# davidesantangelo/krep

Measured on NVIDIA H100. Metric: GB/s scanned (HBM-resident corpus), higher is better.
Workload: dtype u8

## Files before the change

krep_b200/csrc/scan_count.cu:

```cuda
#include <algorithm>
#include "engine.h"
#include "line_rec.cuh"
#include "lit_filters.cuh"

namespace kb {

struct CountDev
{
    LitDevParams p;
    uint64_t own_end;
    uint32_t part_groups, n_parts;
    uint32_t exact;
    uint32_t tail;
    LineRec *recs;
};

struct PartState
{
    uint32_t lines = 0;
    bool has_hit = false, first_open = false, pending = false, seen_nl = false;
    uint64_t covered_to = 0;
};

__device__ __noinline__ unsigned verify_exact_call(const LitDevParams &p, long long cand) { return verify_exact(p, cand); }

__device__ __noinline__ bool scan_for_newline(const LitDevParams &p, uint64_t lo, uint64_t hi)
{
    const uint32_t lane = threadIdx.x & 31;
    if (hi > p.avail_len) hi = p.avail_len;
    for (uint64_t base = lo & ~15ull; base < hi; base += 512)
    {
        const uint64_t unit = base + 16ull * lane;
        uint32_t nm = 0;
        if (unit < hi && unit + 16 > lo)
        {
            if (unit + 16 <= p.avail_len) nm = nl_mask16(__ldg(reinterpret_cast<const uint4 *>(p.text + unit)));
            else
                for (uint64_t q = unit; q < p.avail_len; q++) nm |= (p.text[q] == '\n' ? 1u : 0u) << (uint32_t)(q - unit);
            nm &= range_mask16(unit, lo, hi);
        }
        if (__any_sync(0xffffffffu, nm != 0)) return true;
    }
    return false;
}

__device__ __forceinline__ void settle(const LitDevParams &p, PartState &S, uint64_t upto)
{
    if (S.covered_to < upto && (S.pending || (!S.has_hit && !S.seen_nl)))
        if (scan_for_newline(p, S.covered_to, upto))
        {
            S.pending = false;
            S.seen_nl = true;
        }
}

__device__ __forceinline__ void account(PartState &S, uint32_t hm, uint32_t nm)
{
    const uint32_t lane = threadIdx.x & 31;
    const bool has_nl = nm != 0;
    const uint32_t fnl = has_nl ? (uint32_t)__ffs(nm) - 1 : 0, lnl = has_nl ? 31u - (uint32_t)__clz(nm) : 0;
    const bool f = has_nl && (hm & ((1u << fnl) - 1u)) != 0;
    const bool l = has_nl && ((hm >> lnl) >> 1) != 0;
    uint32_t inner = 0;
    if (__popc(nm) >= 2)
    {
        uint32_t prev = fnl, rest = nm & (nm - 1);
        while (rest)
        {
            const uint32_t nx = (uint32_t)__ffs(rest) - 1;
            if (hm & (((1u << nx) - 1u) & ~((2u << prev) - 1u))) inner++;
            prev = nx;
            rest &= rest - 1;
        }
    }
    const uint32_t A = __ballot_sync(0xffffffffu, has_nl), T = __ballot_sync(0xffffffffu, !has_nl && hm != 0);
    const uint32_t F = __ballot_sync(0xffffffffu, f), Lm = __ballot_sync(0xffffffffu, l);
    uint32_t innersum = 0;
    if (__ballot_sync(0xffffffffu, inner != 0)) innersum = __reduce_add_sync(0xffffffffu, inner);
    if (A == 0)
    {
        if (T)
        {
            if (!S.pending)
            {
                S.lines++;
                if (!S.has_hit && !S.seen_nl) S.first_open = true;
            }
            S.pending = true;
            S.has_hit = true;
        }
        return;
    }
    const uint32_t j1 = (uint32_t)__ffs(A) - 1, jr = 31u - (uint32_t)__clz(A);
    if ((T & ((1u << j1) - 1u)) || ((F >> j1) & 1u))
    {
        if (!S.pending)
        {
            S.lines++;
            if (!S.has_hit && !S.seen_nl) S.first_open = true;
        }
        S.has_hit = true;
    }
    S.pending = false;
    S.seen_nl = true;
    bool gap = false;
    if (has_nl && lane != j1)
    {
        const uint32_t below = A & ((1u << lane) - 1u);
        const uint32_t pj = 31u - (uint32_t)__clz(below);
        const uint32_t between = ((1u << lane) - 1u) & ~((2u << pj) - 1u);
        gap = ((Lm >> pj) & 1u) || (T & between) || f;
    }
    const uint32_t G = __ballot_sync(0xffffffffu, gap);
    S.lines += (uint32_t)__popc(G) + innersum;
    if (G || innersum) S.has_hit = true;
    if (((Lm >> jr) & 1u) || ((T >> jr) >> 1))
    {
        S.lines++;
        S.has_hit = true;
        S.pending = true;
    }
}

__device__ __forceinline__ uint64_t pack_state(const PartState &S)
{
    return (uint64_t)S.lines | ((uint64_t)((S.has_hit ? 1u : 0u) | (S.first_open ? 2u : 0u) | (S.pending ? 4u : 0u) | (S.seen_nl ? 8u : 0u)) << 32);
}
__device__ __forceinline__ void unpack_state(uint64_t k, PartState &S)
{
    S.lines = (uint32_t)k;
    const uint32_t f = (uint32_t)(k >> 32);
    S.has_hit = f & 1u;
    S.first_open = f & 2u;
    S.pending = f & 4u;
    S.seen_nl = f & 8u;
}
__device__ __noinline__ uint64_t account_call(uint64_t packed, uint32_t hm, uint32_t nm)
{
    PartState S;
    unpack_state(packed, S);
    account(S, hm, nm);
    return pack_state(S);
}

template <bool WINDOW>
__device__ __noinline__ uint32_t hit_mask16(const CountDev &D, uint64_t unit, const uint4 &v, uint32_t nx)
{
    const LitDevParams &p = D.p;
    const uint32_t w[5] = {v.x, v.y, v.z, v.w, nx};
    uint32_t hm = 0;
    if (WINDOW)
    {
        const uint32_t mask = p.fold & p.win_mask, k0 = p.K[0];
#pragma unroll
        for (int k = 0; k < 4; k++)
#pragma unroll
            for (int r = 0; r < 4; r++)
            {
                const uint32_t win = r == 0 ? w[k] : __funnelshift_r(w[k], w[k + 1], 8 * r);
                if ((win & mask) == k0)
                {
                    const uint64_t st = unit + 4 * k + r;
                    const bool ok = D.exact ? (st >= p.own_begin && st < p.own_end && st + p.m <= p.avail_len)
                                            : verify_exact_call(p, (long long)st) != 0;
                    if (ok) hm |= 1u << (4 * k + r);
                }
            }
    }
    else
    {
#pragma unroll
        for (int k = 0; k < 4; k++)
#pragma unroll
            for (int d = 0; d < 4; d++)
                if ((w[k] & p.fold) == p.K[d] && verify_exact_call(p, (long long)(unit + 4 * k) - d)) hm |= 1u << (4 * k);
    }
    return hm;
}

__device__ __noinline__ PartState count_tail(const CountDev &D, PartState S, uint64_t cov, uint64_t nl_lo, uint64_t nl_hi, bool window)
{
    const LitDevParams &p = D.p;
    const uint32_t lane = threadIdx.x & 31;
    if (p.avail_len < p.emit_len && cov >= nl_hi) return S;
    const uint64_t last_start = p.avail_len >= p.emit_len ? p.avail_len - p.emit_len : 0;
    uint64_t end = nl_hi > last_start + 1 ? nl_hi : last_start + 1;
    if (!window && end < cov + 1) end = cov + 1;
    for (uint64_t base = cov; base < end; base += 32)
    {
        settle(p, S, base > nl_lo ? base : nl_lo);
        const uint64_t q = base + lane;
        uint32_t hm = 0, nm = 0;
        if (q < end)
        {
            if (p.avail_len >= p.emit_len && q >= p.tail_start && q <= last_start && verify_exact(p, (long long)q)) hm = 1;
            if (!window && q == cov && p.avail_len >= p.emit_len)
                for (uint64_t s = p.tail_start; s < cov && s <= last_start; s++)
                    if (verify_exact(p, (long long)s)) hm = 1;
            if (q >= nl_lo && q < nl_hi && q < p.avail_len && p.text[q] == '\n') nm = 1;
            if (nm) hm = 0;
        }
        account(S, hm, nm);
        S.covered_to = base + 32;
    }
    return S;
}

#ifndef KREP_B200_COUNT_MINB
#define KREP_B200_COUNT_MINB 3
#endif
template <bool WINDOW, bool FOLD, bool MASKED>
__global__ void __launch_bounds__(256, KREP_B200_COUNT_MINB) k_count_lines(const __grid_constant__ CountDev D)
{
    const LitDevParams &p = D.p;
    const uint4 *__restrict__ t4 = reinterpret_cast<const uint4 *>(p.text);
    const uint32_t lane = threadIdx.x & 31;
    const uint32_t warp_global = (blockIdx.x * blockDim.x + threadIdx.x) >> 5, total_warps = (gridDim.x * blockDim.x) >> 5;
    const uint32_t k0 = p.K[0], k1 = p.K[1], k2 = p.K[2], k3 = p.K[3], fold = p.fold, mask = p.win_mask;
    const uint32_t c1 = p.mulc[0], c2 = p.mulc[1], c3 = p.mulc[2];
    for (uint32_t pi = warp_global; pi < D.n_parts; pi += total_warps)
    {
        const uint64_t ga = p.group_begin + (uint64_t)pi * D.part_groups;
        uint64_t gb = ga + D.part_groups;
        if (gb > p.group_end) gb = p.group_end;
        const bool last_part = pi + 1 == D.n_parts;
        const uint64_t nl_lo = ga * 16 > p.own_begin ? ga * 16 : p.own_begin;
        const uint64_t nl_hi = (last_part || gb * 16 > D.own_end) ? D.own_end : gb * 16;
        PartState S;
        S.covered_to = nl_lo;
        for (uint64_t g = ga; g < gb; g += 128)
        {
            uint4 v[4];
            uint32_t nx[4];
            bool ok[4];
#pragma unroll
            for (int u = 0; u < 4; u++)
            {
                const uint64_t gi = g + 32 * u + lane;
                ok[u] = gi < gb;
                v[u] = ok[u] ? ld_stream(t4 + gi) : make_uint4(0u, 0u, 0u, 0u);
                nx[u] = 0;
                if (WINDOW && ok[u] && (lane == 31 || gi + 1 >= gb)) nx[u] = __ldg(reinterpret_cast<const uint32_t *>(t4 + gi + 1));
            }
            uint32_t cand = 0;
#pragma unroll
            for (int u = 0; u < 4; u++)
            {
                bool h;
                if (WINDOW)
                {
                    const uint32_t nb = __shfl_down_sync(0xffffffffu, v[u].x, 1);
                    if (!(lane == 31 || g + 32 * u + lane + 1 >= gb)) nx[u] = nb;
                    h = hit_vec_w<FOLD, MASKED>(v[u], nx[u], fold, mask, k0, c1, c2, c3);
                }
                else
                    h = hit_vec<FOLD>(v[u], fold, k0, k1, k2, k3);
                cand |= (h && ok[u]) ? (1u << u) : 0u;
            }
            const uint32_t any = __reduce_or_sync(0xffffffffu, cand);
            if (any)
            {
                const uint64_t tile_lo = g * 16;
                settle(p, S, tile_lo > nl_lo ? tile_lo : nl_lo);
                const bool inside = tile_lo >= nl_lo && tile_lo + 2048 <= nl_hi;
                uint64_t st = pack_state(S);
#pragma unroll
                for (int u = 0; u < 4; u++)
                {
                    const uint64_t unit = tile_lo + 512ull * u + 16ull * lane;
                    uint32_t hm = 0, nm = 0;
                    if (ok[u])
                    {
                        if ((cand >> u) & 1u) hm = hit_mask16<WINDOW>(D, unit, v[u], nx[u]);
                        nm = nl_mask16(v[u]);
                        if (!inside) nm &= range_mask16(unit, nl_lo, nl_hi);
                    }
                    st = account_call(st, hm, nm);
                }
                unpack_state(st, S);
                S.covered_to = tile_lo + 2048;
            }
        }
        if (last_part && D.tail) S = count_tail(D, S, gb * 16, nl_lo, nl_hi, WINDOW);
        uint32_t flags = 0;
        if (S.has_hit)
        {
            if (S.pending && S.covered_to < nl_hi && scan_for_newline(p, S.covered_to, nl_hi)) S.pending = false;
            flags = LR_HAS_HIT | (S.first_open ? LR_FIRST_OPEN : 0u) | (S.pending ? LR_LAST_PENDING : 0u) | LR_HAS_NL;
        }
        else
        {
            const bool nl = S.seen_nl || (S.covered_to < nl_hi && scan_for_newline(p, S.covered_to, nl_hi));
            flags = nl ? LR_HAS_NL : 0u;
        }
        if (lane == 0) D.recs[pi] = LineRec{S.lines, flags};
    }
}

__global__ void __launch_bounds__(1024) k_count_finish(const LineRec *recs, uint32_t n, uint64_t *d_out, uint64_t *h_out)
{
    __shared__ uint64_t s_lines[1024];
    __shared__ uint32_t s_flags[1024];
    const uint32_t per = (n + blockDim.x - 1) / blockDim.x;
    const uint32_t a = threadIdx.x * per, b = a + per < n ? a + per : n;
    uint64_t lines = 0;
    uint32_t flags = 0;
    for (uint32_t i = a; i < b; i++) append_rec(lines, flags, recs[i].lines, recs[i].flags);
    s_lines[threadIdx.x] = lines;
    s_flags[threadIdx.x] = flags;
    __syncthreads();
    if (threadIdx.x == 0)
    {
        lines = 0;
        flags = 0;
        for (uint32_t t = 0; t < blockDim.x; t++) append_rec(lines, flags, s_lines[t], s_flags[t]);
        d_out[0] = lines;
        d_out[1] = flags;
        h_out[0] = lines;
        h_out[1] = flags;
    }
}

#define CKC(call)                                                                                  \
    do                                                                                             \
    {                                                                                              \
        cudaError_t e_ = (call);                                                                   \
        if (e_ != cudaSuccess)                                                                     \
        {                                                                                          \
            set_error(-2, "CUDA error %s at %s:%d (%s)", cudaGetErrorName(e_), __FILE__, __LINE__, \
                      cudaGetErrorString(e_));                                                     \
            return -2;                                                                             \
        }                                                                                          \
    } while (0)

bool count_lines_eligible(const Plan *plan, const search_params_t *P, int algo)
{
    if (!P->count_lines_mode || plan->is_regex || plan->whole_word == 2) return false;
    if (plan->is_ac)
    {
        for (const std::string &s : plan->patterns)
            if (s.find('\n') != std::string::npos) return false;
        return true;
    }
    if (plan->emit_len != plan->m) return false;
    if (plan->pattern.find('\n') != std::string::npos) return false;
    return algo == KREP_B200_ALGO_BMH || algo == KREP_B200_ALGO_KMP || algo == KREP_B200_ALGO_MEMCHR ||
           algo == KREP_B200_ALGO_MEMCHR_SHORT || algo == KREP_B200_ALGO_SSE42;
}

int ensure_line_out(DevCtx &E, uint64_t n)
{
    if (n <= E.line_out_cap) return 0;
    CKC(cudaDeviceSynchronize());
    cudaFree(E.d_line_out);
    cudaFreeHost(E.h_line_out);
    E.d_line_out = nullptr;
    E.h_line_out = nullptr;
    E.line_out_cap = 0;
    uint64_t cap = 64;
    while (cap < n) cap *= 2;
    CKC(cudaMalloc(&E.d_line_out, cap * 2 * sizeof(uint64_t)));
    CKC(cudaHostAlloc(&E.h_line_out, cap * 2 * sizeof(uint64_t), cudaHostAllocMapped | cudaHostAllocPortable));
    E.line_out_cap = cap;
    return 0;
}

int launch_count_lines(DevCtx &E, const Plan *plan, const krep_b200_shard_t *sh, cudaStream_t stream, uint64_t index)
{
    if (((uintptr_t)sh->d_text & 15) != 0)
    {
        set_error(-3, "shard text pointer must be 16-byte aligned");
        return -3;
    }
    const PlanDev *pd = plan_on_device(plan, E);
    if (!pd) return -2;
    if (ensure_line_out(E, index + 1) != 0) return -2;
    if (plan->is_ac)
    {
        const int slot = set_count_slot(E);
        const int rc = set_count_begin(E, plan, sh, stream, slot);
        return rc != 0 ? rc : set_count_end(E, plan, sh, stream, slot, index);
    }
    CountDev D;
    memset(&D, 0, sizeof D);
    LitDevParams &p = D.p;
    const uint64_t own_end = sh->own_end < sh->avail_len ? sh->own_end : sh->avail_len;
    p.text = (const uint8_t *)sh->d_text;
    p.avail_len = sh->avail_len;
    p.own_begin = sh->own_begin;
    p.own_end = own_end;
    p.global_offset = sh->global_offset;
    p.prev_byte = sh->prev_byte;
    p.next_byte = sh->next_byte;
    uint64_t total_groups;
    const bool window = plan->filter == FILTER_WINDOW4;
    if (!window)
    {
        total_groups = sh->avail_len / 16;
        p.tail_start = total_groups ? total_groups * 16 - 3 : 0;
    }
    else
    {
        total_groups = sh->avail_len >= 20 ? (sh->avail_len - 20) / 16 + 1 : 0;
        p.tail_start = total_groups * 16;
    }
    p.group_begin = sh->own_begin / 16;
    p.group_end = (own_end + 2) / 16 + 1;
    D.tail = p.group_end > total_groups ? 1u : 0u;
    if (p.group_end > total_groups) p.group_end = total_groups;
    if (p.group_begin > p.group_end) p.group_begin = p.group_end;
    p.m = plan->m;
    p.emit_len = plan->emit_len;
    for (int d = 0; d < 4; d++) p.K[d] = plan->K[d];
    p.fold = plan->fold;
    p.win_mask = plan->win_mask;
    p.mulc[0] = 1u << 24;
    p.mulc[1] = 1u << 16;
    p.mulc[2] = 1u << 8;
    p.pat_val = pd->d_pat_val;
    p.pat_mask = pd->d_pat_mask;
    p.whole_word = plan->whole_word;
    D.own_end = own_end;
    {
        bool letters = true;
        for (unsigned char ch : plan->pattern) letters &= is_alpha_c(ch);
        D.exact = (window && plan->m <= 4 && plan->whole_word == 0 && (plan->case_sensitive || letters)) ? 1u : 0u;
    }
    const uint64_t groups = p.group_end - p.group_begin;
    const char *v = getenv("KREP_B200_COUNT_PART_KB");
    const uint32_t kb_ = v && atoi(v) > 0 ? (uint32_t)atoi(v) : 64;
    uint64_t part = std::max<uint32_t>(128, kb_ * 64 / 128 * 128);
    const uint64_t max_parts = 1u << 18;
    if ((groups + part - 1) / part > max_parts) part = ((groups + max_parts - 1) / max_parts + 127) / 128 * 128;
    D.part_groups = (uint32_t)part;
    D.n_parts = (uint32_t)std::max<uint64_t>((groups + part - 1) / part, 1);
    if (D.n_parts > E.line_recs_cap)
    {
        CKC(cudaStreamSynchronize(stream));
        cudaFree(E.d_line_recs);
        E.d_line_recs = nullptr;
        E.line_recs_cap = 0;
        const uint64_t cap = std::max<uint64_t>(D.n_parts, 1u << 16);
        CKC(cudaMalloc(&E.d_line_recs, cap * sizeof(LineRec)));
        E.line_recs_cap = cap;
    }
    D.recs = (LineRec *)E.d_line_recs;
    const bool folded = plan->fold != 0xFFFFFFFFu, masked = plan->win_mask != 0xFFFFFFFFu;
    const uint64_t want_blocks = ((uint64_t)D.n_parts + 7) / 8;
    const unsigned grid = (unsigned)std::min<uint64_t>(want_blocks, (uint64_t)E.sm_count * KREP_B200_COUNT_MINB);
    if (!window)
    {
        if (folded) k_count_lines<false, true, false><<<grid, 256, 0, stream>>>(D);
        else k_count_lines<false, false, false><<<grid, 256, 0, stream>>>(D);
    }
    else if (folded)
    {
        if (masked) k_count_lines<true, true, true><<<grid, 256, 0, stream>>>(D);
        else k_count_lines<true, true, false><<<grid, 256, 0, stream>>>(D);
    }
    else
    {
        if (masked) k_count_lines<true, false, true><<<grid, 256, 0, stream>>>(D);
        else k_count_lines<true, false, false><<<grid, 256, 0, stream>>>(D);
    }
    CKC(cudaGetLastError());
    k_count_finish<<<1, 1024, 0, stream>>>(D.recs, D.n_parts, E.d_line_out + 2 * index, E.h_line_out + 2 * index);
    CKC(cudaGetLastError());
    count_launch(2);
    return 0;
}

uint64_t combine_line_records(const uint64_t *recs, size_t n)
{
    uint64_t lines = 0;
    uint32_t flags = 0;
    for (size_t i = 0; i < n; i++) append_rec(lines, flags, recs[2 * i], (uint32_t)recs[2 * i + 1]);
    return lines;
}

}
```

Before: 3123.

## Rewrite line counting with a bitwise carry-propagation formula and prefetch loads

Replaces the branchy per-warp line-accounting state machine, including its newline rescans and packed-state noinline calls, with a compact carry-based formula. Per-lane hit masks are combined with newline masks through an addition trick, and the carry between lanes and iterations comes from ballots. The loop also double-buffers the next tile's vector loads, computes window hits as full masks, and verifies candidates bit by bit. Tiles with no hits only run a cheap newline test. This cuts instruction count and serialization in the count kernel, but relies on subtle bit arithmetic that must match the old semantics at part boundaries.

```diff
diff --git a/krep_b200/csrc/scan_count.cu b/krep_b200/csrc/scan_count.cu
--- a/krep_b200/csrc/scan_count.cu
+++ b/krep_b200/csrc/scan_count.cu
@@ -9,176 +9,103 @@
 {
     LitDevParams p;
     uint64_t own_end;
+    uint64_t hit_hi;
     uint32_t part_groups, n_parts;
     uint32_t exact;
     uint32_t tail;
     LineRec *recs;
 };
 
-struct PartState
-{
-    uint32_t lines = 0;
-    bool has_hit = false, first_open = false, pending = false, seen_nl = false;
-    uint64_t covered_to = 0;
+struct CountState
+{
+    uint32_t lines;
+    uint32_t carry;
+    uint32_t seen;
+    uint32_t first_open;
 };
 
 __device__ __noinline__ unsigned verify_exact_call(const LitDevParams &p, long long cand) { return verify_exact(p, cand); }
 
-__device__ __noinline__ bool scan_for_newline(const LitDevParams &p, uint64_t lo, uint64_t hi)
-{
-    const uint32_t lane = threadIdx.x & 31;
-    if (hi > p.avail_len) hi = p.avail_len;
-    for (uint64_t base = lo & ~15ull; base < hi; base += 512)
-    {
-        const uint64_t unit = base + 16ull * lane;
-        uint32_t nm = 0;
-        if (unit < hi && unit + 16 > lo)
+__device__ __forceinline__ void account(CountState &S, uint32_t hm, uint32_t nm, uint32_t lanes_below)
+{
+    const uint32_t ev = hm | nm;
+    const uint32_t E = __ballot_sync(0xffffffffu, ev != 0);
+    const uint32_t N = __ballot_sync(0xffffffffu, nm > hm);
+    const uint32_t eb = E & lanes_below, nb = N & lanes_below;
+    const uint32_t cin = eb ? (nb > (eb ^ nb) ? 1u : 0u) : S.carry;
+    S.lines += __popc((((nm << 1) | cin) + (~ev & 0xFFFFu)) & hm);
+    if (E != 0 && !S.seen)
+    {
+        const uint32_t F = __ballot_sync(0xffffffffu, (ev & (0u - ev) & hm) != 0);
+        S.first_open = (F & E & (0u - E)) ? 1u : 0u;
+        S.seen = 1;
+    }
+    S.carry = E ? (N > (E ^ N) ? 1u : 0u) : S.carry;
+}
+
+__device__ __forceinline__ bool has_nl16(const uint4 &v)
+{
+    const uint32_t x0 = v.x ^ 0x0A0A0A0Au, x1 = v.y ^ 0x0A0A0A0Au, x2 = v.z ^ 0x0A0A0A0Au, x3 = v.w ^ 0x0A0A0A0Au;
+    const uint32_t z = ((x0 - 0x01010101u) & ~x0) | ((x1 - 0x01010101u) & ~x1) | ((x2 - 0x01010101u) & ~x2) |
+                       ((x3 - 0x01010101u) & ~x3);
+    return (z & 0x80808080u) != 0;
+}
+
+template <bool FOLD, bool MASKED>
+__device__ __forceinline__ uint32_t window_hits16(const uint4 &v, uint32_t nx, uint32_t fold, uint32_t mask, uint32_t k0,
+                                                  uint32_t c1, uint32_t c2, uint32_t c3)
+{
+    uint32_t w[5] = {v.x, v.y, v.z, v.w, nx};
+    uint32_t hm = 0;
+#pragma unroll
+    for (int k = 0; k < 4; k++)
+    {
+        uint32_t lo = w[k], hi = w[k + 1];
+        if (FOLD)
         {
-            if (unit + 16 <= p.avail_len) nm = nl_mask16(__ldg(reinterpret_cast<const uint4 *>(p.text + unit)));
-            else
-                for (uint64_t q = unit; q < p.avail_len; q++) nm |= (p.text[q] == '\n' ? 1u : 0u) << (uint32_t)(q - unit);
-            nm &= range_mask16(unit, lo, hi);
+            lo &= fold;
+            hi &= fold;
         }
-        if (__any_sync(0xffffffffu, nm != 0)) return true;
-    }
-    return false;
-}
-
-__device__ __forceinline__ void settle(const LitDevParams &p, PartState &S, uint64_t upto)
-{
-    if (S.covered_to < upto && (S.pending || (!S.has_hit && !S.seen_nl)))
-        if (scan_for_newline(p, S.covered_to, upto))
+        uint32_t x0 = lo, x1 = hi * c1 + __umulhi(lo, c1), x2 = hi * c2 + __umulhi(lo, c2), x3 = hi * c3 + __umulhi(lo, c3);
+        if (MASKED)
         {
-            S.pending = false;
-            S.seen_nl = true;
+            x0 &= mask; x1 &= mask; x2 &= mask; x3 &= mask;
         }
-}
-
-__device__ __forceinline__ void account(PartState &S, uint32_t hm, uint32_t nm)
-{
-    const uint32_t lane = threadIdx.x & 31;
-    const bool has_nl = nm != 0;
-    const uint32_t fnl = has_nl ? (uint32_t)__ffs(nm) - 1 : 0, lnl = has_nl ? 31u - (uint32_t)__clz(nm) : 0;
-    const bool f = has_nl && (hm & ((1u << fnl) - 1u)) != 0;
-    const bool l = has_nl && ((hm >> lnl) >> 1) != 0;
-    uint32_t inner = 0;
-    if (__popc(nm) >= 2)
-    {
-        uint32_t prev = fnl, rest = nm & (nm - 1);
-        while (rest)
-        {
-            const uint32_t nx = (uint32_t)__ffs(rest) - 1;
-            if (hm & (((1u << nx) - 1u) & ~((2u << prev) - 1u))) inner++;
-            prev = nx;
-            rest &= rest - 1;
-        }
-    }
-    const uint32_t A = __ballot_sync(0xffffffffu, has_nl), T = __ballot_sync(0xffffffffu, !has_nl && hm != 0);
-    const uint32_t F = __ballot_sync(0xffffffffu, f), Lm = __ballot_sync(0xffffffffu, l);
-    uint32_t innersum = 0;
-    if (__ballot_sync(0xffffffffu, inner != 0)) innersum = __reduce_add_sync(0xffffffffu, inner);
-    if (A == 0)
-    {
-        if (T)
-        {
-            if (!S.pending)
-            {
-                S.lines++;
-                if (!S.has_hit && !S.seen_nl) S.first_open = true;
-            }
-            S.pending = true;
-            S.has_hit = true;
-        }
-        return;
-    }
-    const uint32_t j1 = (uint32_t)__ffs(A) - 1, jr = 31u - (uint32_t)__clz(A);
-    if ((T & ((1u << j1) - 1u)) || ((F >> j1) & 1u))
-    {
-        if (!S.pending)
-        {
-            S.lines++;
-            if (!S.has_hit && !S.seen_nl) S.first_open = true;
-        }
-        S.has_hit = true;
-    }
-    S.pending = false;
-    S.seen_nl = true;
-    bool gap = false;
-    if (has_nl && lane != j1)
-    {
-        const uint32_t below = A & ((1u << lane) - 1u);
-        const uint32_t pj = 31u - (uint32_t)__clz(below);
-        const uint32_t between = ((1u << lane) - 1u) & ~((2u << pj) - 1u);
-        gap = ((Lm >> pj) & 1u) || (T & between) || f;
-    }
-    const uint32_t G = __ballot_sync(0xffffffffu, gap);
-    S.lines += (uint32_t)__popc(G) + innersum;
-    if (G || innersum) S.has_hit = true;
-    if (((Lm >> jr) & 1u) || ((T >> jr) >> 1))
-    {
-        S.lines++;
-        S.has_hit = true;
-        S.pending = true;
-    }
-}
-
-__device__ __forceinline__ uint64_t pack_state(const PartState &S)
-{
-    return (uint64_t)S.lines | ((uint64_t)((S.has_hit ? 1u : 0u) | (S.first_open ? 2u : 0u) | (S.pending ? 4u : 0u) | (S.seen_nl ? 8u : 0u)) << 32);
-}
-__device__ __forceinline__ void unpack_state(uint64_t k, PartState &S)
-{
-    S.lines = (uint32_t)k;
-    const uint32_t f = (uint32_t)(k >> 32);
-    S.has_hit = f & 1u;
-    S.first_open = f & 2u;
-    S.pending = f & 4u;
-    S.seen_nl = f & 8u;
-}
-__device__ __noinline__ uint64_t account_call(uint64_t packed, uint32_t hm, uint32_t nm)
-{
-    PartState S;
-    unpack_state(packed, S);
-    account(S, hm, nm);
-    return pack_state(S);
+        hm |= ((x0 == k0) ? 1u : 0u) << (4 * k) | ((x1 == k0) ? 2u : 0u) << (4 * k) | ((x2 == k0) ? 4u : 0u) << (4 * k) |
+              ((x3 == k0) ? 8u : 0u) << (4 * k);
+    }
+    return hm;
+}
+
+template <bool FOLD>
+__device__ __forceinline__ uint32_t aligned_cands16(const uint4 &v, uint32_t fold, uint32_t k0, uint32_t k1, uint32_t k2, uint32_t k3)
+{
+    const uint32_t w[4] = {v.x, v.y, v.z, v.w};
+    uint32_t cm = 0;
+#pragma unroll
+    for (int k = 0; k < 4; k++)
+    {
+        const uint32_t x = FOLD ? w[k] & fold : w[k];
+        cm |= ((x == k0 ? 1u : 0u) | (x == k1 ? 2u : 0u) | (x == k2 ? 4u : 0u) | (x == k3 ? 8u : 0u)) << (4 * k);
+    }
+    return cm;
 }
 
 template <bool WINDOW>
-__device__ __noinline__ uint32_t hit_mask16(const CountDev &D, uint64_t unit, const uint4 &v, uint32_t nx)
-{
-    const LitDevParams &p = D.p;
-    const uint32_t w[5] = {v.x, v.y, v.z, v.w, nx};
+__device__ __forceinline__ uint32_t verified_hits16(const LitDevParams &p, uint64_t unit, uint32_t cm)
+{
     uint32_t hm = 0;
-    if (WINDOW)
-    {
-        const uint32_t mask = p.fold & p.win_mask, k0 = p.K[0];
-#pragma unroll
-        for (int k = 0; k < 4; k++)
-#pragma unroll
-            for (int r = 0; r < 4; r++)
-            {
-                const uint32_t win = r == 0 ? w[k] : __funnelshift_r(w[k], w[k + 1], 8 * r);
-                if ((win & mask) == k0)
-                {
-                    const uint64_t st = unit + 4 * k + r;
-                    const bool ok = D.exact ? (st >= p.own_begin && st < p.own_end && st + p.m <= p.avail_len)
-                                            : verify_exact_call(p, (long long)st) != 0;
-                    if (ok) hm |= 1u << (4 * k + r);
-                }
-            }
-    }
-    else
-    {
-#pragma unroll
-        for (int k = 0; k < 4; k++)
-#pragma unroll
-            for (int d = 0; d < 4; d++)
-                if ((w[k] & p.fold) == p.K[d] && verify_exact_call(p, (long long)(unit + 4 * k) - d)) hm |= 1u << (4 * k);
+    while (cm)
+    {
+        const uint32_t b = (uint32_t)__ffs(cm) - 1;
+        cm &= cm - 1;
+        const long long st = WINDOW ? (long long)(unit + b) : (long long)(unit + (b & ~3u)) - (long long)(b & 3u);
+        if (verify_exact_call(p, st)) hm |= 1u << (WINDOW ? b : b & ~3u);
     }
     return hm;
 }
 
-__device__ __noinline__ PartState count_tail(const CountDev &D, PartState S, uint64_t cov, uint64_t nl_lo, uint64_t nl_hi, bool window)
+__device__ __noinline__ CountState count_tail(const CountDev &D, CountState S, uint64_t cov, uint64_t nl_lo, uint64_t nl_hi, bool window)
 {
     const LitDevParams &p = D.p;
     const uint32_t lane = threadIdx.x & 31;
@@ -188,7 +115,6 @@
     if (!window && end < cov + 1) end = cov + 1;
     for (uint64_t base = cov; base < end; base += 32)
     {
-        settle(p, S, base > nl_lo ? base : nl_lo);
         const uint64_t q = base + lane;
         uint32_t hm = 0, nm = 0;
         if (q < end)
@@ -200,8 +126,7 @@
             if (q >= nl_lo && q < nl_hi && q < p.avail_len && p.text[q] == '\n') nm = 1;
             if (nm) hm = 0;
         }
-        account(S, hm, nm);
-        S.covered_to = base + 32;
+        account(S, hm, nm, (1u << lane) - 1u);
     }
     return S;
 }
@@ -214,10 +139,11 @@
 {
     const LitDevParams &p = D.p;
     const uint4 *__restrict__ t4 = reinterpret_cast<const uint4 *>(p.text);
-    const uint32_t lane = threadIdx.x & 31;
+    const uint32_t lane = threadIdx.x & 31, lanes_below = (1u << lane) - 1u;
     const uint32_t warp_global = (blockIdx.x * blockDim.x + threadIdx.x) >> 5, total_warps = (gridDim.x * blockDim.x) >> 5;
     const uint32_t k0 = p.K[0], k1 = p.K[1], k2 = p.K[2], k3 = p.K[3], fold = p.fold, mask = p.win_mask;
     const uint32_t c1 = p.mulc[0], c2 = p.mulc[1], c3 = p.mulc[2];
+    const bool exact = WINDOW && D.exact;
     for (uint32_t pi = warp_global; pi < D.n_parts; pi += total_warps)
     {
         const uint64_t ga = p.group_begin + (uint64_t)pi * D.part_groups;
@@ -226,74 +152,68 @@
         const bool last_part = pi + 1 == D.n_parts;
         const uint64_t nl_lo = ga * 16 > p.own_begin ? ga * 16 : p.own_begin;
         const uint64_t nl_hi = (last_part || gb * 16 > D.own_end) ? D.own_end : gb * 16;
-        PartState S;
-        S.covered_to = nl_lo;
+        const uint64_t in_hi = nl_hi < D.hit_hi ? nl_hi : D.hit_hi;
+        CountState S{0u, 1u, 0u, 0u};
+        uint4 nv[4];
+#pragma unroll
+        for (int u = 0; u < 4; u++)
+        {
+            const uint64_t gi = ga + 32 * u + lane;
+            nv[u] = gi < gb ? ld_stream(t4 + gi) : make_uint4(0u, 0u, 0u, 0u);
+        }
         for (uint64_t g = ga; g < gb; g += 128)
         {
             uint4 v[4];
-            uint32_t nx[4];
-            bool ok[4];
+#pragma unroll
+            for (int u = 0; u < 4; u++) v[u] = nv[u];
 #pragma unroll
             for (int u = 0; u < 4; u++)
             {
-                const uint64_t gi = g + 32 * u + lane;
-                ok[u] = gi < gb;
-                v[u] = ok[u] ? ld_stream(t4 + gi) : make_uint4(0u, 0u, 0u, 0u);
-                nx[u] = 0;
-                if (WINDOW && ok[u] && (lane == 31 || gi + 1 >= gb)) nx[u] = __ldg(reinterpret_cast<const uint32_t *>(t4 + gi + 1));
+                const uint64_t gi = g + 128 + 32 * u + lane;
+                nv[u] = gi < gb ? ld_stream(t4 + gi) : make_uint4(0u, 0u, 0u, 0u);
             }
-            uint32_t cand = 0;
+            const uint64_t tile_lo = g * 16;
+            const bool inside = g + 128 <= gb && tile_lo >= nl_lo && tile_lo + 2048 <= in_hi;
 #pragma unroll
             for (int u = 0; u < 4; u++)
             {
-                bool h;
+                const uint64_t gi = g + 32 * u + lane, unit = gi * 16;
+                const bool ok = gi < gb;
+                uint32_t cm;
+                uint32_t nx = 0;
                 if (WINDOW)
                 {
                     const uint32_t nb = __shfl_down_sync(0xffffffffu, v[u].x, 1);
-                    if (!(lane == 31 || g + 32 * u + lane + 1 >= gb)) nx[u] = nb;
-                    h = hit_vec_w<FOLD, MASKED>(v[u], nx[u], fold, mask, k0, c1, c2, c3);
+                    nx = (lane == 31 || gi + 1 >= gb) ? (ok ? __ldg(reinterpret_cast<const uint32_t *>(t4 + gi + 1)) : 0u) : nb;
+                    cm = ok ? window_hits16<FOLD, MASKED>(v[u], nx, fold, mask, k0, c1, c2, c3) : 0u;
+                    if (exact && !inside) cm &= range_mask16(unit, p.own_begin, D.hit_hi);
                 }
                 else
-                    h = hit_vec<FOLD>(v[u], fold, k0, k1, k2, k3);
-                cand |= (h && ok[u]) ? (1u << u) : 0u;
-            }
-            const uint32_t any = __reduce_or_sync(0xffffffffu, cand);
-            if (any)
-            {
-                const uint64_t tile_lo = g * 16;
-                settle(p, S, tile_lo > nl_lo ? tile_lo : nl_lo);
-                const bool inside = tile_lo >= nl_lo && tile_lo + 2048 <= nl_hi;
-                uint64_t st = pack_state(S);
-#pragma unroll
-                for (int u = 0; u < 4; u++)
+                    cm = (ok && hit_vec<FOLD>(v[u], fold, k0, k1, k2, k3)) ? 1u : 0u;
+                if (!inside || __any_sync(0xffffffffu, cm != 0))
                 {
-                    const uint64_t unit = tile_lo + 512ull * u + 16ull * lane;
-                    uint32_t hm = 0, nm = 0;
-                    if (ok[u])
+                    uint32_t nm = nl_mask16(v[u]);
+                    if (!inside) nm &= range_mask16(unit, nl_lo, nl_hi);
+                    uint32_t hm = cm;
+                    if (!exact)
                     {
-                        if ((cand >> u) & 1u) hm = hit_mask16<WINDOW>(D, unit, v[u], nx[u]);
-                        nm = nl_mask16(v[u]);
-                        if (!inside) nm &= range_mask16(unit, nl_lo, nl_hi);
+                        if (!WINDOW && cm) cm = aligned_cands16<FOLD>(v[u], fold, k0, k1, k2, k3);
+                        hm = verified_hits16<WINDOW>(p, unit, cm);
                     }
-                    st = account_call(st, hm, nm);
+                    account(S, hm, nm, lanes_below);
                 }
-                unpack_state(st, S);
-                S.covered_to = tile_lo + 2048;
+                else if (__any_sync(0xffffffffu, has_nl16(v[u])))
+                {
+                    S.carry = 1;
+                    S.seen = 1;
+                }
             }
         }
         if (last_part && D.tail) S = count_tail(D, S, gb * 16, nl_lo, nl_hi, WINDOW);
-        uint32_t flags = 0;
-        if (S.has_hit)
-        {
-            if (S.pending && S.covered_to < nl_hi && scan_for_newline(p, S.covered_to, nl_hi)) S.pending = false;
-            flags = LR_HAS_HIT | (S.first_open ? LR_FIRST_OPEN : 0u) | (S.pending ? LR_LAST_PENDING : 0u) | LR_HAS_NL;
-        }
-        else
-        {
-            const bool nl = S.seen_nl || (S.covered_to < nl_hi && scan_for_newline(p, S.covered_to, nl_hi));
-            flags = nl ? LR_HAS_NL : 0u;
-        }
-        if (lane == 0) D.recs[pi] = LineRec{S.lines, flags};
+        const uint32_t lines = __reduce_add_sync(0xffffffffu, S.lines);
+        uint32_t flags = S.seen ? LR_HAS_NL : 0u;
+        if (lines) flags |= LR_HAS_HIT | (S.first_open ? LR_FIRST_OPEN : 0u) | (S.carry ? 0u : LR_LAST_PENDING);
+        if (lane == 0) D.recs[pi] = LineRec{lines, flags};
     }
 }
 
@@ -421,6 +341,7 @@
     p.pat_mask = pd->d_pat_mask;
     p.whole_word = plan->whole_word;
     D.own_end = own_end;
+    D.hit_hi = std::min<uint64_t>(own_end, sh->avail_len >= plan->m ? sh->avail_len - plan->m + 1 : 0);
     {
         bool letters = true;
         for (unsigned char ch : plan->pattern) letters &= is_alpha_c(ch);
```

New measurement: 3118 (median of 6 runs). Within noise of the previous version (-0.1%).
